# mcmilk/7-Zip-zstd

Hardware: NVIDIA H100
Metric: zstd-L3 encode+decode throughput (higher is better)
Workload: dtype u8

## Files before the change

### 7-zip-zstd_b200/csrc/zstd_enc_dp.cu

```cuda
#include "b2z_device.cuh"
#include "b2z_kernels.h"
#include "b2z_zstd_cost.h"

namespace b2z {

constexpr uint32_t DP_RING = 32;
static_assert(DP_RING > B2Z_CAP && (DP_RING & (DP_RING - 1u)) == 0, "the ring holds cost[i + 1 .. i + B2Z_CAP] while cost[i] is written");
struct DpWarpSmem {
    uint32_t ring[DP_RING][32];
    uint32_t candTile[32][33];
    uint32_t srcTile[32][9];
    uint32_t chcTile[32][9];
    uint8_t litc[256];
};

enum { DPC_HIST, DPC_DP_LOAD, DPC_DP, DPC_DP_STORE, DPC_CNT_LOAD, DPC_CNT, DPC_SCAN, DPC_EMIT_LOAD, DPC_EMIT, DPC_N };
#ifdef B2Z_DP_CLOCKS
__device__ unsigned long long dp_clocks[DPC_N + 1];
#define DP_TICK(ph) do { const long long now_ = clock64(); dpc[ph] += (unsigned long long)(now_ - dpLast); dpLast = now_; } while (0)
#define DP_CLOCKS_FLUSH() do { if (lane == 0) { for (int p_ = 0; p_ < DPC_N; p_++) atomicAdd(&dp_clocks[p_], dpc[p_]); atomicAdd(&dp_clocks[DPC_N], 1ull); } } while (0)
#else
#define DP_TICK(ph) do { } while (0)
#define DP_CLOCKS_FLUSH() do { } while (0)
#endif

__device__ __forceinline__ uint32_t dp_log16(uint32_t x) {
    const uint32_t hb = highbit32(x);
    const uint32_t k = hb >= 4u ? ((x >> (hb - 4u)) & 15u) : ((x << (4u - hb)) & 15u);
    const uint64_t lo = 0x0908070605030201ull, hi = 0x100F0F0E0D0C0B0Aull;
    const uint32_t fr = (uint32_t)(((k < 8u ? lo : hi) >> ((k & 7u) * 8u)) & 0xFFu);
    return 16u * hb + ((k == 0u && (x & (x - 1u)) == 0u) ? 0u : fr);
}

__device__ __forceinline__ void dp_fetch_cand(uint32_t (&r)[32], const uint32_t* __restrict__ base, uint32_t bn, uint32_t t, uint32_t lane) {
#pragma unroll
    for (uint32_t j = 0; j < 32u; j++) {
        const uint32_t pos = j * B2Z_SEG + 32u * t + lane;
        r[j] = pos < bn ? __ldcs(base + pos) : 0u;
    }
}
__device__ __forceinline__ void dp_put_cand(DpWarpSmem& sm, const uint32_t (&r)[32], uint32_t lane) {
#pragma unroll
    for (uint32_t j = 0; j < 32u; j++) sm.candTile[j][lane] = r[j];
}
__device__ __forceinline__ void dp_fetch_bytes(uint32_t (&r)[8], const uint8_t* __restrict__ base, uint32_t bn, uint32_t t, uint32_t lane) {
#pragma unroll
    for (uint32_t k = 0; k < 8u; k++) {
        const uint32_t row = 4u * k + (lane >> 3), wd = lane & 7u, pos = row * B2Z_SEG + 32u * t + 4u * wd;
        r[k] = pos < bn ? __ldg(reinterpret_cast<const uint32_t*>(base + pos)) : 0u;
    }
}
__device__ __forceinline__ void dp_put_bytes(uint32_t (*tile)[9], const uint32_t (&r)[8], uint32_t lane) {
#pragma unroll
    for (uint32_t k = 0; k < 8u; k++) tile[4u * k + (lane >> 3)][lane & 7u] = r[k];
}
__device__ __forceinline__ void dp_store_byte_tile(const uint32_t (*tile)[9], uint8_t* __restrict__ base, uint32_t bn, uint32_t t, uint32_t lane) {
#pragma unroll
    for (uint32_t r = 0; r < 8u; r++) {
        const uint32_t row = 4u * r + (lane >> 3), wd = lane & 7u, pos = row * B2Z_SEG + 32u * t + 4u * wd;
        if (pos < bn) *reinterpret_cast<uint32_t*>(base + pos) = tile[row][wd];
    }
}

static_assert(DP_RING == 32u && B2Z_DP_NTRUNC < 4u && (uint64_t)B2Z_SEG * B2Z_DP_LIT_MAX + 1024u < (1u << 29),
              "ring slot = position in the tile; k fits two bits; a cost fits 29 bits");
__device__ __forceinline__ void dp_match(const DpWarpSmem& sm, uint32_t lane, uint32_t p, uint32_t lim, uint32_t& mc, uint32_t& mh) {
    const uint32_t c = sm.candTile[lane][p];
    const uint32_t len = B2Z_CAND_LEN(c), ob = 16u * highbit32(B2Z_CAND_OFF(c) + 3u) + B2Z_DP_MATCH;
    uint32_t m = 0xFFFFFFFFu;
#pragma unroll
    for (uint32_t k = 0; k <= B2Z_DP_NTRUNC; k++) {
        const uint32_t key = ((ob + sm.ring[(p + len - k) & (DP_RING - 1u)][lane]) << 2) | k;
        m = (len >= B2Z_DP_MINLEN + k && key < m) ? key : m;
    }
    mc = p >= lim ? 0u : m >> 2;
    mh = p >= lim ? 0u : len - (m & 3u);
}

struct DpWalk {
    uint32_t i, ns, nl, lastEnd;
    uint32_t rep0, rep1, rep2, prevEnd;
};

__device__ __forceinline__ uint32_t dp_nonzero_mask(const uint32_t* row) {
    uint32_t m = 0;
#pragma unroll
    for (int k = 0; k < 8; k++) {
        const uint32_t w = row[k];
        const uint32_t f = ((((w & 0x7F7F7F7Fu) + 0x7F7F7F7Fu) | w) & 0x80808080u) >> 7;
        m |= ((f * 0x00204081u) >> 21 & 15u) << (4 * k);
    }
    return m;
}

template <bool EMIT>
__device__ __forceinline__ uint32_t dp_walk_tile(DpWarpSmem& sm, DpWalk& k, uint32_t t, uint32_t lane, uint32_t sn, uint32_t s0 ,
                                             const uint64_t* __restrict__ fw , uint32_t segAbs , uint32_t nWords,
                                             const uint32_t* __restrict__ cnd ,
                                             uint64_t* __restrict__ outSeq) {
    const uint32_t tEnd = (32u * t + 32u) < sn ? (32u * t + 32u) : sn;
    uint32_t lits = 0;
    if (k.i >= tEnd) return lits;
    const uint32_t inTile = tEnd - 32u * t;
    const uint32_t M = dp_nonzero_mask(sm.chcTile[lane]) & (inTile >= 32u ? 0xFFFFFFFFu : ((1u << inTile) - 1u));
    while (k.i < tEnd) {
        uint32_t w = k.i & 31u;
        const uint32_t rem = M >> w;
        const uint32_t r = rem ? (uint32_t)(__ffs((int)rem) - 1) : (tEnd - k.i);
        if (r) {
            if (EMIT) lits |= (0xFFFFFFFFu >> (32u - r)) << w;
            k.nl += r; k.i += r; w += r;
            if (!rem) break;
        }
        uint32_t l = (sm.chcTile[lane][w >> 2] >> (8u * (w & 3u))) & 255u;
        const uint32_t off = EMIT ? B2Z_CAND_OFF(sm.candTile[lane][w]) : 0u;
        if (l == B2Z_CAP) {
            const uint32_t o = EMIT ? off : B2Z_CAND_OFF(__ldg(cnd + k.i));
            l = match_len(fw, segAbs + k.i - o, segAbs + k.i, sn - k.i, nWords);
        }
        if (EMIT) {
            const uint32_t pos = s0 + k.i, ll = pos - k.prevEnd;
            uint32_t code = 0, offBase;
            if (ll) { if (off == k.rep0) code = 1; else if (off == k.rep1) code = 2; else if (off == k.rep2) code = 3; }
            else { if (off == k.rep1) code = 1; else if (off == k.rep2) code = 2; else if (k.rep0 > 1u && off == k.rep0 - 1u) code = 3; }
            if (code == 0) { offBase = off + 3u; k.rep2 = k.rep1; k.rep1 = k.rep0; k.rep0 = off; }
            else {
                offBase = code;
                const uint32_t idx = code - 1u + (ll == 0u);
                if (idx != 0) {
                    const uint32_t cur = idx == 3 ? k.rep0 - 1u : (idx == 1 ? k.rep1 : k.rep2);
                    if (idx != 1) k.rep2 = k.rep1;
                    k.rep1 = k.rep0; k.rep0 = cur;
                }
            }
            outSeq[k.ns] = B2Z_PACK_SEQ(offBase, ll, l);
            k.prevEnd = pos + l;
        }
        k.ns++; k.i += l; k.lastEnd = s0 + k.i;
    }
    return lits;
}

__device__ __forceinline__ void dp_emit_literals(const DpWarpSmem& sm, uint32_t lits, uint32_t dst, uint32_t lane, uint8_t* __restrict__ out) {
    const uint32_t below = (1u << lane) - 1u;
    for (uint32_t L = 0; L < 32u; L++) {
        const uint32_t m = __shfl_sync(B2Z_FULL, lits, L), d = __shfl_sync(B2Z_FULL, dst, L);
        if (m >> lane & 1u) out[d + __popc(m & below)] = (uint8_t)(sm.srcTile[L][lane >> 2] >> (8u * (lane & 3u)));
    }
}

__global__ void __launch_bounds__(B2Z_DP_WARPS * 32)
zstd_enc_dp_kernel(const uint8_t* __restrict__ src, uint64_t srcSize, EncGeom g, const uint32_t* __restrict__ cand, uint8_t* __restrict__ choice,
                   uint64_t* __restrict__ seqs, uint32_t* __restrict__ nseq, uint8_t* __restrict__ lits, uint32_t* __restrict__ nlit,
                   uint32_t nBlockSlots) {
    B2Z_DYN_SMEM(DpWarpSmem, allSm);
    const uint32_t lane = threadIdx.x & 31u, wib = threadIdx.x >> 5;
    DpWarpSmem& sm = allSm[wib];
    const uint32_t bw = blockIdx.x * B2Z_DP_WARPS + wib;
    if (bw >= nBlockSlots) return;
    const uint32_t bpf = 1u << (g.frameLog - 17u);
    const uint64_t f = bw >> (g.frameLog - 17u);
    const uint32_t b = bw & (bpf - 1u);
    const uint32_t n = enc_frame_bytes(g, srcSize, f);
    const uint32_t b0 = b << 17;
    if (b0 >= n) return;
    const uint32_t bn = (n - b0) < B2Z_BLOCK ? (n - b0) : B2Z_BLOCK;
    const uint64_t f0 = f << g.frameLog;
    const uint8_t* __restrict__ fb = src + f0;
    const uint8_t* __restrict__ bs = fb + b0;
    const uint32_t* __restrict__ cndB = cand + f0 + b0;
    uint8_t* __restrict__ chcB = choice + f0 + b0;
    uint64_t* __restrict__ out = seqs + (size_t)bw * B2Z_MAXSEQ;
    uint8_t* __restrict__ lit = lits + f0 + b0;
    const uint32_t nTiles = ((bn < B2Z_SEG ? bn : B2Z_SEG) + 31u) >> 5;
#ifdef B2Z_DP_CLOCKS
    unsigned long long dpc[DPC_N] = {};
    long long dpLast = clock64();
#endif

    uint32_t* const hist = &sm.candTile[0][0];
    for (uint32_t i = lane; i < 256u; i += 32u) hist[i] = 0;
    __syncwarp();
    for (uint32_t idx = lane;; idx += 32u) {
        const uint32_t o = (idx >> 2) * 256u + (idx & 3u) * 16u;
        if ((idx & ~31u) * 64u >= bn) break;
        if (o + 16u <= bn) {
            const uint4 q = __ldg(reinterpret_cast<const uint4*>(bs + o));
            const uint32_t ws[4] = { q.x, q.y, q.z, q.w };
#pragma unroll
            for (int k = 0; k < 4; k++) { atomicAdd(&hist[ws[k] & 255u], 1u); atomicAdd(&hist[(ws[k] >> 8) & 255u], 1u); atomicAdd(&hist[(ws[k] >> 16) & 255u], 1u); atomicAdd(&hist[ws[k] >> 24], 1u); }
        } else for (uint32_t k = o; k < bn && k < o + 16u; k++) atomicAdd(&hist[bs[k]], 1u);
    }
    __syncwarp();
    {
        uint32_t part = 0;
#pragma unroll
        for (int k = 0; k < 8; k++) part += hist[lane * 8u + k];
#pragma unroll
        for (int d = 16; d; d >>= 1) part += __shfl_xor_sync(B2Z_FULL, part, d);
        const uint32_t lt = dp_log16(part);
#pragma unroll
        for (int k = 0; k < 8; k++) {
            const uint32_t h = hist[lane * 8u + k];
            uint32_t v = B2Z_DP_LIT_MAX;
            if (h) { const uint32_t lh = dp_log16(h); v = lt > lh ? lt - lh : 1u; }
            sm.litc[lane * 8u + k] = (uint8_t)(v < B2Z_DP_LIT_MIN ? B2Z_DP_LIT_MIN : (v > B2Z_DP_LIT_MAX ? B2Z_DP_LIT_MAX : v));
        }
    }
    __syncwarp();
    DP_TICK(DPC_HIST);

    const uint32_t s0 = lane * B2Z_SEG;
    const bool active = s0 < bn;
    const uint32_t sn = active ? ((bn - s0) < B2Z_SEG ? (bn - s0) : B2Z_SEG) : 0u;
    uint32_t diff = 0;
    const uint32_t first = bs[0];
    const uint32_t first4 = first * 0x01010101u;
    uint32_t c1 = 0;
    if (active) sm.ring[sn & (DP_RING - 1u)][lane] = 0;
    uint32_t cr[32], sr[8];
    dp_fetch_cand(cr, cndB, bn, nTiles - 1u, lane);
    dp_fetch_bytes(sr, bs, bn, nTiles - 1u, lane);
    for (uint32_t t = nTiles; t-- > 0;) {
        dp_put_cand(sm, cr, lane);
        dp_put_bytes(sm.srcTile, sr, lane);
        if (t) { dp_fetch_cand(cr, cndB, bn, t - 1u, lane); dp_fetch_bytes(sr, bs, bn, t - 1u, lane); }
        __syncwarp();
        DP_TICK(DPC_DP_LOAD);
        if (32u * t < sn) {
            const uint32_t lim = sn - 32u * t;
            uint32_t mc[4], mh[4];
#pragma unroll
            for (uint32_t j = 0; j < 4u; j++) dp_match(sm, lane, 31u - j, lim, mc[j], mh[j]);
#pragma unroll 2
            for (int wi = 7; wi >= 0; wi--) {
                const uint32_t b4 = sm.srcTile[lane][wi];
                const int inWord = (int)lim - 4 * wi;
                const uint32_t x = b4 ^ first4;
                diff |= inWord >= 4 ? x : (inWord > 0 ? x & ((1u << (8 * inWord)) - 1u) : 0u);
                uint32_t packed = 0;
#pragma unroll
                for (uint32_t j = 0; j < 4u; j++) {
                    const uint32_t p = 4u * (uint32_t)wi + 3u - j, sh = 8u * (3u - j);
                    const uint32_t lc = c1 + sm.litc[(b4 >> sh) & 255u];
                    c1 = lc < mc[j] ? lc : mc[j];
                    packed |= (mc[j] < lc ? mh[j] : 0u) << sh;
                    sm.ring[p][lane] = c1;
                    if (wi > 0) dp_match(sm, lane, p - 4u, lim, mc[j], mh[j]);
                }
                sm.chcTile[lane][wi] = packed;
            }
        }
        __syncwarp();
        DP_TICK(DPC_DP);
        dp_store_byte_tile(sm.chcTile, chcB, bn, t, lane);
        DP_TICK(DPC_DP_STORE);
    }
    if (!__any_sync(B2Z_FULL, diff != 0u) && bn > 1u) {
        if (lane == 0) { out[0] = B2Z_PACK_SEQ(1u + 3u, 1u, bn - 1u); lit[0] = bs[0]; nseq[bw] = 1u; nlit[bw] = 1u; }
        DP_CLOCKS_FLUSH();
        return;
    }

    const uint64_t* __restrict__ fw = reinterpret_cast<const uint64_t*>(fb);
    const uint32_t nWords = (n + 7u) >> 3;
    const uint32_t* __restrict__ cnd = cndB + s0;
    DpWalk k; k.i = 0; k.ns = 0; k.nl = 0; k.lastEnd = 0; k.rep0 = k.rep1 = k.rep2 = 0; k.prevEnd = 0;
    uint32_t qr[8];
    for (uint32_t t = 0; t < nTiles; t++) {
        if (t) { dp_put_bytes(sm.chcTile, qr, lane); __syncwarp(); }
        if (t + 1u < nTiles) dp_fetch_bytes(qr, chcB, bn, t + 1u, lane);
        DP_TICK(DPC_CNT_LOAD);
        dp_walk_tile<false>(sm, k, t, lane, sn, s0, fw, b0 + s0, nWords, cnd, nullptr);
        __syncwarp();
        DP_TICK(DPC_CNT);
    }
    const uint32_t cntSeq = k.ns, cntLit = k.nl;
    uint32_t seqBase = cntSeq, litBase = cntLit, prevEnd = cntSeq ? k.lastEnd : 0u;
#pragma unroll
    for (int d = 1; d < 32; d <<= 1) {
        const uint32_t a = __shfl_up_sync(B2Z_FULL, seqBase, d), c = __shfl_up_sync(B2Z_FULL, litBase, d), e = __shfl_up_sync(B2Z_FULL, prevEnd, d);
        if (lane >= (uint32_t)d) { seqBase += a; litBase += c; prevEnd = e > prevEnd ? e : prevEnd; }
    }
    const uint32_t totSeq = __shfl_sync(B2Z_FULL, seqBase, 31), totLit = __shfl_sync(B2Z_FULL, litBase, 31);
    seqBase -= cntSeq; litBase -= cntLit;
    prevEnd = __shfl_up_sync(B2Z_FULL, prevEnd, 1); if (lane == 0) prevEnd = 0;
    DP_TICK(DPC_SCAN);
    k.i = 0; k.ns = 0; k.nl = 0; k.prevEnd = prevEnd;
    dp_fetch_bytes(qr, chcB, bn, 0, lane);
    dp_fetch_bytes(sr, bs, bn, 0, lane);
    dp_fetch_cand(cr, cndB, bn, 0, lane);
    for (uint32_t t = 0; t < nTiles; t++) {
        dp_put_bytes(sm.chcTile, qr, lane);
        dp_put_bytes(sm.srcTile, sr, lane);
        dp_put_cand(sm, cr, lane);
        if (t + 1u < nTiles) { dp_fetch_bytes(qr, chcB, bn, t + 1u, lane); dp_fetch_bytes(sr, bs, bn, t + 1u, lane); dp_fetch_cand(cr, cndB, bn, t + 1u, lane); }
        __syncwarp();
        DP_TICK(DPC_EMIT_LOAD);
        const uint32_t litAt = litBase + k.nl;
        const uint32_t lits = dp_walk_tile<true>(sm, k, t, lane, sn, s0, fw, b0 + s0, nWords, cnd, out + seqBase);
        dp_emit_literals(sm, lits, litAt, lane, lit);
        __syncwarp();
        DP_TICK(DPC_EMIT);
    }
    if (lane == 0) { nseq[bw] = totSeq; nlit[bw] = totLit; }
    DP_CLOCKS_FLUSH();
}

#ifndef B2Z_CUEMU
size_t zstd_enc_dp_smem_bytes() { return sizeof(DpWarpSmem) * B2Z_DP_WARPS; }

cudaError_t launch_zstd_enc_dp(const uint8_t* src, uint64_t srcSize, const EncGeom& g, const uint32_t* cand, uint8_t* choice,
                               uint64_t* seqs, uint32_t* nseq, uint8_t* lits, uint32_t* nlit, cudaStream_t st) {
    if (srcSize == 0) return cudaSuccess;
    const uint64_t F = 1ull << g.frameLog, nFrames = (srcSize + F - 1) >> g.frameLog;
    const uint32_t nBlockSlots = (uint32_t)(nFrames << (g.frameLog - 17u));
    cudaError_t e = cudaFuncSetAttribute(zstd_enc_dp_kernel, cudaFuncAttributeMaxDynamicSharedMemorySize, (int)zstd_enc_dp_smem_bytes());
    if (e != cudaSuccess) return e;
    zstd_enc_dp_kernel<<<(nBlockSlots + B2Z_DP_WARPS - 1) / B2Z_DP_WARPS, B2Z_DP_WARPS * 32, zstd_enc_dp_smem_bytes(), st>>>(
        src, srcSize, g, cand, choice, seqs, nseq, lits, nlit, nBlockSlots);
    return cudaGetLastError();
}
#endif

#if defined(B2Z_DP_CLOCKS) && !defined(B2Z_CUEMU)
extern "C" int b200z_dp_clocks(unsigned long long* out) {
    static const unsigned long long zero[DPC_N + 1] = {};
    cudaError_t e = cudaMemcpyFromSymbol(out, dp_clocks, sizeof(dp_clocks));
    if (e == cudaSuccess) e = cudaMemcpyToSymbol(dp_clocks, zero, sizeof(dp_clocks));
    return (int)e;
}
#endif

}
```

Measured before the change: 30390.

## Walk DP choices once, staging sequences per lane and compacting afterwards

```diff
diff --git a/7-zip-zstd_b200/csrc/zstd_enc_dp.cu b/7-zip-zstd_b200/csrc/zstd_enc_dp.cu
--- a/7-zip-zstd_b200/csrc/zstd_enc_dp.cu
+++ b/7-zip-zstd_b200/csrc/zstd_enc_dp.cu
@@ -6,15 +6,23 @@
 
 constexpr uint32_t DP_RING = 32;
 static_assert(DP_RING > B2Z_CAP && (DP_RING & (DP_RING - 1u)) == 0, "the ring holds cost[i + 1 .. i + B2Z_CAP] while cost[i] is written");
+constexpr uint32_t DP_LANE_SEQS = B2Z_SEG / B2Z_DP_MINLEN;
+static_assert(32u * DP_LANE_SEQS <= B2Z_MAXSEQ, "every lane's records fit its staging run in the block's sequence array");
+constexpr uint32_t DP_PEND = 16;
+static_assert(32u / B2Z_DP_MINLEN <= DP_PEND / 2u, "a tile's records fit behind the ones a lane may still hold");
 struct DpWarpSmem {
-    uint32_t ring[DP_RING][32];
+    union {
+        uint32_t ring[DP_RING][32];
+        uint64_t recs[32][DP_PEND];
+        uint32_t runs[3][33];
+    };
     uint32_t candTile[32][33];
     uint32_t srcTile[32][9];
     uint32_t chcTile[32][9];
     uint8_t litc[256];
 };
 
-enum { DPC_HIST, DPC_DP_LOAD, DPC_DP, DPC_DP_STORE, DPC_CNT_LOAD, DPC_CNT, DPC_SCAN, DPC_EMIT_LOAD, DPC_EMIT, DPC_N };
+enum { DPC_HIST, DPC_DP_LOAD, DPC_DP, DPC_DP_STORE, DPC_WALK_LOAD, DPC_WALK, DPC_WALK_STORE, DPC_SCAN, DPC_MOVE, DPC_LIT_LOAD, DPC_LIT, DPC_N };
 #ifdef B2Z_DP_CLOCKS
 __device__ unsigned long long dp_clocks[DPC_N + 1];
 #define DP_TICK(ph) do { const long long now_ = clock64(); dpc[ph] += (unsigned long long)(now_ - dpLast); dpLast = now_; } while (0)
@@ -43,11 +51,13 @@
 #pragma unroll
     for (uint32_t j = 0; j < 32u; j++) sm.candTile[j][lane] = r[j];
 }
+template <bool WRITTEN = false>
 __device__ __forceinline__ void dp_fetch_bytes(uint32_t (&r)[8], const uint8_t* __restrict__ base, uint32_t bn, uint32_t t, uint32_t lane) {
 #pragma unroll
     for (uint32_t k = 0; k < 8u; k++) {
         const uint32_t row = 4u * k + (lane >> 3), wd = lane & 7u, pos = row * B2Z_SEG + 32u * t + 4u * wd;
-        r[k] = pos < bn ? __ldg(reinterpret_cast<const uint32_t*>(base + pos)) : 0u;
+        const uint32_t* const p = reinterpret_cast<const uint32_t*>(base + pos);
+        r[k] = pos < bn ? (WRITTEN ? __ldcg(p) : __ldg(p)) : 0u;
     }
 }
 __device__ __forceinline__ void dp_put_bytes(uint32_t (*tile)[9], const uint32_t (&r)[8], uint32_t lane) {
@@ -78,8 +88,8 @@
 }
 
 struct DpWalk {
-    uint32_t i, ns, nl, lastEnd;
-    uint32_t rep0, rep1, rep2, prevEnd;
+    uint32_t i, ns, nl, np;
+    uint32_t prevEnd, rep0, rep1, rep2;
 };
 
 __device__ __forceinline__ uint32_t dp_nonzero_mask(const uint32_t* row) {
@@ -93,11 +103,8 @@
     return m;
 }
 
-template <bool EMIT>
-__device__ __forceinline__ uint32_t dp_walk_tile(DpWarpSmem& sm, DpWalk& k, uint32_t t, uint32_t lane, uint32_t sn, uint32_t s0 ,
-                                             const uint64_t* __restrict__ fw , uint32_t segAbs , uint32_t nWords,
-                                             const uint32_t* __restrict__ cnd ,
-                                             uint64_t* __restrict__ outSeq) {
+__device__ __forceinline__ uint32_t dp_walk_tile(DpWarpSmem& sm, DpWalk& k, uint32_t t, uint32_t lane, uint32_t sn,
+                                                 const uint64_t* __restrict__ fw , uint32_t segAbs , uint32_t nWords) {
     const uint32_t tEnd = (32u * t + 32u) < sn ? (32u * t + 32u) : sn;
     uint32_t lits = 0;
     if (k.i >= tEnd) return lits;
@@ -108,37 +115,43 @@
         const uint32_t rem = M >> w;
         const uint32_t r = rem ? (uint32_t)(__ffs((int)rem) - 1) : (tEnd - k.i);
         if (r) {
-            if (EMIT) lits |= (0xFFFFFFFFu >> (32u - r)) << w;
+            lits |= (0xFFFFFFFFu >> (32u - r)) << w;
             k.nl += r; k.i += r; w += r;
             if (!rem) break;
         }
         uint32_t l = (sm.chcTile[lane][w >> 2] >> (8u * (w & 3u))) & 255u;
-        const uint32_t off = EMIT ? B2Z_CAND_OFF(sm.candTile[lane][w]) : 0u;
-        if (l == B2Z_CAP) {
-            const uint32_t o = EMIT ? off : B2Z_CAND_OFF(__ldg(cnd + k.i));
-            l = match_len(fw, segAbs + k.i - o, segAbs + k.i, sn - k.i, nWords);
-        }
-        if (EMIT) {
-            const uint32_t pos = s0 + k.i, ll = pos - k.prevEnd;
-            uint32_t code = 0, offBase;
-            if (ll) { if (off == k.rep0) code = 1; else if (off == k.rep1) code = 2; else if (off == k.rep2) code = 3; }
-            else { if (off == k.rep1) code = 1; else if (off == k.rep2) code = 2; else if (k.rep0 > 1u && off == k.rep0 - 1u) code = 3; }
-            if (code == 0) { offBase = off + 3u; k.rep2 = k.rep1; k.rep1 = k.rep0; k.rep0 = off; }
-            else {
-                offBase = code;
-                const uint32_t idx = code - 1u + (ll == 0u);
-                if (idx != 0) {
-                    const uint32_t cur = idx == 3 ? k.rep0 - 1u : (idx == 1 ? k.rep1 : k.rep2);
-                    if (idx != 1) k.rep2 = k.rep1;
-                    k.rep1 = k.rep0; k.rep0 = cur;
-                }
+        const uint32_t off = B2Z_CAND_OFF(sm.candTile[lane][w]);
+        if (l == B2Z_CAP) l = match_len(fw, segAbs + k.i - off, segAbs + k.i, sn - k.i, nWords);
+        const uint32_t ll = k.i - k.prevEnd;
+        uint32_t code = 0, offBase;
+        if (ll) { if (off == k.rep0) code = 1; else if (off == k.rep1) code = 2; else if (off == k.rep2) code = 3; }
+        else { if (off == k.rep1) code = 1; else if (off == k.rep2) code = 2; else if (k.rep0 > 1u && off == k.rep0 - 1u) code = 3; }
+        if (code == 0) { offBase = off + 3u; k.rep2 = k.rep1; k.rep1 = k.rep0; k.rep0 = off; }
+        else {
+            offBase = code;
+            const uint32_t idx = code - 1u + (ll == 0u);
+            if (idx != 0) {
+                const uint32_t cur = idx == 3 ? k.rep0 - 1u : (idx == 1 ? k.rep1 : k.rep2);
+                if (idx != 1) k.rep2 = k.rep1;
+                k.rep1 = k.rep0; k.rep0 = cur;
             }
-            outSeq[k.ns] = B2Z_PACK_SEQ(offBase, ll, l);
-            k.prevEnd = pos + l;
-        }
-        k.ns++; k.i += l; k.lastEnd = s0 + k.i;
+        }
+        sm.recs[lane][k.np ^ (lane & 15u)] = B2Z_PACK_SEQ(offBase, ll, l);
+        k.np++; k.ns++; k.i += l; k.prevEnd = k.i;
     }
     return lits;
+}
+
+__device__ __forceinline__ void dp_store_records(const DpWarpSmem& sm, DpWalk& k, uint32_t lane, uint64_t* __restrict__ out) {
+    static_assert(DP_PEND == 16u, "a half-warp stores one lane's run");
+    const uint32_t from = DP_LANE_SEQS * lane + k.ns - k.np, r = lane & 15u;
+#pragma unroll 4
+    for (uint32_t s = 0; s < 16u; s++) {
+        const uint32_t L = 2u * s + (lane >> 4);
+        const uint32_t cnt = __shfl_sync(B2Z_FULL, k.np, L), at = __shfl_sync(B2Z_FULL, from, L);
+        if (r < cnt) out[at + r] = sm.recs[L][r ^ (L & 15u)];
+    }
+    k.np = 0;
 }
 
 __device__ __forceinline__ void dp_emit_literals(const DpWarpSmem& sm, uint32_t lits, uint32_t dst, uint32_t lane, uint8_t* __restrict__ out) {
@@ -149,7 +162,7 @@
     }
 }
 
-__global__ void __launch_bounds__(B2Z_DP_WARPS * 32)
+__global__ void __launch_bounds__(B2Z_DP_WARPS * 32, 4)
 zstd_enc_dp_kernel(const uint8_t* __restrict__ src, uint64_t srcSize, EncGeom g, const uint32_t* __restrict__ cand, uint8_t* __restrict__ choice,
                    uint64_t* __restrict__ seqs, uint32_t* __restrict__ nseq, uint8_t* __restrict__ lits, uint32_t* __restrict__ nlit,
                    uint32_t nBlockSlots) {
@@ -264,19 +277,21 @@
 
     const uint64_t* __restrict__ fw = reinterpret_cast<const uint64_t*>(fb);
     const uint32_t nWords = (n + 7u) >> 3;
-    const uint32_t* __restrict__ cnd = cndB + s0;
-    DpWalk k; k.i = 0; k.ns = 0; k.nl = 0; k.lastEnd = 0; k.rep0 = k.rep1 = k.rep2 = 0; k.prevEnd = 0;
+    DpWalk k; k.i = 0; k.ns = 0; k.nl = 0; k.np = 0; k.prevEnd = 0; k.rep0 = k.rep1 = k.rep2 = 0;
     uint32_t qr[8];
     for (uint32_t t = 0; t < nTiles; t++) {
-        if (t) { dp_put_bytes(sm.chcTile, qr, lane); __syncwarp(); }
-        if (t + 1u < nTiles) dp_fetch_bytes(qr, chcB, bn, t + 1u, lane);
-        DP_TICK(DPC_CNT_LOAD);
-        dp_walk_tile<false>(sm, k, t, lane, sn, s0, fw, b0 + s0, nWords, cnd, nullptr);
-        __syncwarp();
-        DP_TICK(DPC_CNT);
+        if (t) { dp_put_bytes(sm.chcTile, qr, lane); dp_put_cand(sm, cr, lane); __syncwarp(); }
+        if (t + 1u < nTiles) { dp_fetch_bytes(qr, chcB, bn, t + 1u, lane); dp_fetch_cand(cr, cndB, bn, t + 1u, lane); }
+        DP_TICK(DPC_WALK_LOAD);
+        sm.srcTile[lane][t & 7u] = dp_walk_tile(sm, k, t, lane, sn, fw, b0 + s0, nWords);
+        __syncwarp();
+        DP_TICK(DPC_WALK);
+        if ((t & 7u) == 7u || t + 1u == nTiles) dp_store_byte_tile(sm.srcTile, chcB, bn, t & ~7u, lane);
+        if (__any_sync(B2Z_FULL, k.np > DP_PEND / 2u) || t + 1u == nTiles) { dp_store_records(sm, k, lane, out); __syncwarp(); }
+        DP_TICK(DPC_WALK_STORE);
     }
     const uint32_t cntSeq = k.ns, cntLit = k.nl;
-    uint32_t seqBase = cntSeq, litBase = cntLit, prevEnd = cntSeq ? k.lastEnd : 0u;
+    uint32_t seqBase = cntSeq, litBase = cntLit, prevEnd = cntSeq ? s0 + k.prevEnd : 0u;
 #pragma unroll
     for (int d = 1; d < 32; d <<= 1) {
         const uint32_t a = __shfl_up_sync(B2Z_FULL, seqBase, d), c = __shfl_up_sync(B2Z_FULL, litBase, d), e = __shfl_up_sync(B2Z_FULL, prevEnd, d);
@@ -285,23 +300,52 @@
     const uint32_t totSeq = __shfl_sync(B2Z_FULL, seqBase, 31), totLit = __shfl_sync(B2Z_FULL, litBase, 31);
     seqBase -= cntSeq; litBase -= cntLit;
     prevEnd = __shfl_up_sync(B2Z_FULL, prevEnd, 1); if (lane == 0) prevEnd = 0;
+    sm.runs[0][lane] = seqBase; sm.runs[1][lane] = DP_LANE_SEQS * lane - seqBase; sm.runs[2][lane] = s0 - prevEnd;
+    if (lane == 0) sm.runs[0][32] = totSeq;
+    __syncwarp();
     DP_TICK(DPC_SCAN);
-    k.i = 0; k.ns = 0; k.nl = 0; k.prevEnd = prevEnd;
-    dp_fetch_bytes(qr, chcB, bn, 0, lane);
+    {
+        constexpr uint32_t U = 8;
+        uint32_t L = 0;
+        for (uint32_t c = 0; c < totSeq; c += 32u * U) {
+            uint64_t v[U];
+            uint32_t patch[U];
+#pragma unroll
+            for (uint32_t u = 0; u < U; u++) {
+                const uint32_t r = c + 32u * u + lane;
+                patch[u] = 0;
+                if (r < totSeq) {
+                    while (sm.runs[0][L + 1u] <= r) L++;
+                    v[u] = __ldcg(out + r + sm.runs[1][L]);
+                    if (r == sm.runs[0][L]) patch[u] = sm.runs[2][L];
+                }
+            }
+            __syncwarp();
+#pragma unroll
+            for (uint32_t u = 0; u < U; u++) {
+                const uint32_t r = c + 32u * u + lane;
+                if (r < totSeq) out[r] = v[u] + ((uint64_t)patch[u] << 28);
+            }
+        }
+    }
+    DP_TICK(DPC_MOVE);
+    uint32_t litAt = litBase;
     dp_fetch_bytes(sr, bs, bn, 0, lane);
-    dp_fetch_cand(cr, cndB, bn, 0, lane);
+    dp_fetch_bytes<true>(qr, chcB, bn, 0, lane);
     for (uint32_t t = 0; t < nTiles; t++) {
-        dp_put_bytes(sm.chcTile, qr, lane);
+        if ((t & 7u) == 0u) {
+            dp_put_bytes(sm.chcTile, qr, lane);
+            if (t + 8u < nTiles) dp_fetch_bytes<true>(qr, chcB, bn, t + 8u, lane);
+        }
         dp_put_bytes(sm.srcTile, sr, lane);
-        dp_put_cand(sm, cr, lane);
-        if (t + 1u < nTiles) { dp_fetch_bytes(qr, chcB, bn, t + 1u, lane); dp_fetch_bytes(sr, bs, bn, t + 1u, lane); dp_fetch_cand(cr, cndB, bn, t + 1u, lane); }
-        __syncwarp();
-        DP_TICK(DPC_EMIT_LOAD);
-        const uint32_t litAt = litBase + k.nl;
-        const uint32_t lits = dp_walk_tile<true>(sm, k, t, lane, sn, s0, fw, b0 + s0, nWords, cnd, out + seqBase);
+        if (t + 1u < nTiles) dp_fetch_bytes(sr, bs, bn, t + 1u, lane);
+        __syncwarp();
+        DP_TICK(DPC_LIT_LOAD);
+        const uint32_t lits = sm.chcTile[lane][t & 7u];
         dp_emit_literals(sm, lits, litAt, lane, lit);
-        __syncwarp();
-        DP_TICK(DPC_EMIT);
+        litAt += __popc(lits);
+        __syncwarp();
+        DP_TICK(DPC_LIT);
     }
     if (lane == 0) { nseq[bw] = totSeq; nlit[bw] = totLit; }
     DP_CLOCKS_FLUSH();
```

New measurement: 32020, median of 6. +5.4%, better.
